# huzaifakhan04/truely-real-time-ai-generated-video-detection-framework-for-social-platforms

Hardware: AMD Instinct MI355X
Metric: frames/sec (detect+embed+drift) 720p (higher is better)
Workload: dtype f32

## Files before the change

### truely-real-time-ai-generated-video-detection-framework-for-social-platforms_amd/csrc/trl_api.hip

```cpp
#include <stdarg.h>
#include <stdio.h>
#include <string.h>
#include <stdlib.h>

#include "trl_ctx.h"

static thread_local char g_err[512] = "";
int g_trl_no_fnconv = 0;
int g_trl_pnet_gate = 0;

#include <mutex>
namespace {
std::mutex g_gate_mu;
hipEvent_t g_gate_ev[64] = {};
bool g_gate_set[64] = {};
}
int trl_gate_wait(trl_ctx* c, hipStream_t s) {
    const int d = c->cfg.device;
    if (!g_trl_pnet_gate || d < 0 || d >= 64) return TRL_OK;
    std::lock_guard<std::mutex> lk(g_gate_mu);
    if (g_gate_set[d]) TRL_HIP(hipStreamWaitEvent(s, g_gate_ev[d], 0));
    return TRL_OK;
}
int trl_gate_record(trl_ctx* c, hipStream_t s) {
    const int d = c->cfg.device;
    if (!g_trl_pnet_gate || d < 0 || d >= 64) return TRL_OK;
    std::lock_guard<std::mutex> lk(g_gate_mu);
    if (!g_gate_ev[d]) TRL_HIP(hipEventCreateWithFlags(&g_gate_ev[d], hipEventDisableTiming));
    TRL_HIP(hipEventRecord(g_gate_ev[d], s));
    g_gate_set[d] = true;
    return TRL_OK;
}
void trl_set_error(const char* fmt, ...) {
    va_list ap;
    va_start(ap, fmt);
    vsnprintf(g_err, sizeof g_err, fmt, ap);
    va_end(ap);
}

extern "C" {

int trl_abi_version(void) { return TRL_ABI_VERSION; }
const char* trl_last_error(void) { return g_err; }

int trl_default_config(trl_config* cfg) {
    if (!cfg) return TRL_ERR_INVALID;
    cfg->device = 0;
    cfg->min_face_size = 20;
    cfg->thr0 = 0.6f; cfg->thr1 = 0.7f; cfg->thr2 = 0.7f;
    cfg->factor = 0.709;
    cfg->cap_level = 2048;
    cfg->cap_frame = 2048;
    cfg->max_faces = 64;
    cfg->pnet_mode = 0;
    cfg->embed_mode = 0;
    cfg->embed_precision = 0;
    return TRL_OK;
}

int trl_create(const trl_config* cfg, trl_ctx** out) {
    if (!cfg || !out) { trl_set_error("null argument"); return TRL_ERR_INVALID; }
    if (cfg->cap_level < 64 || cfg->cap_level > (1 << 24) || cfg->cap_frame < 64 || cfg->cap_frame > (1 << 24) || (cfg->cap_level & 3) ||
        (cfg->cap_frame & 3) || cfg->min_face_size < 12 || cfg->max_faces < 1 || !(cfg->factor > 0.1 && cfg->factor < 0.99) || cfg->embed_mode < 0 || cfg->embed_mode > 3 ||
        cfg->embed_precision < 0 || cfg->embed_precision > 2) {
        trl_set_error("bad trl_config (list start capacities must be multiples of 4 in [64, 2^24], min_face_size >= 12)");
        return TRL_ERR_INVALID;
    }
    TRL_HIP(hipSetDevice(cfg->device));
    trl_ctx* c = new trl_ctx();
    c->cfg = *cfg;
    c->pnet_prof = trl_tune_set("TRL_PNET_CLOCK");
    if (hipMalloc((void**)&c->pnet_clk, 8 * 41) != hipSuccess || hipMemset(c->pnet_clk, 0, 8 * 41) != hipSuccess || hipMemset(c->pnet_clk, 0xFF, 8) != hipSuccess ||
        hipMalloc((void**)&c->pnet_cursor, 64) != hipSuccess || hipHostMalloc((void**)&c->h_pinned, 1024) != hipSuccess ||
        hipEventCreate(&c->ev_call0) != hipSuccess || hipEventCreate(&c->ev_call1) != hipSuccess) {
        trl_set_error("context allocation failed: %s", hipGetErrorString(hipGetLastError()));
        trl_destroy(c);
        return TRL_ERR_HIP;
    }
    memset(c->h_pinned, 0, 1024);
    *out = c;
    return TRL_OK;
}

int trl_destroy(trl_ctx* c) {
    if (!c) return TRL_OK;
    (void)hipSetDevice(c->cfg.device);
    (void)hipDeviceSynchronize();
    c->pend.active = false;
    for (auto& kv : c->W) if (kv.second.pt) (void)hipFree(kv.second.pt);
    if (c->wdev) (void)hipFree(c->wdev);
    if (c->arena.base) (void)hipFree(c->arena.base);
    if (c->scratch.base) (void)hipFree(c->scratch.base);
    if (c->sims_tmp.base) (void)hipFree(c->sims_tmp.base);
    if (c->pyr_tab) (void)hipFree(c->pyr_tab);
    for (auto& b : c->fn_cap) if (b.p) (void)hipFree(b.p);
    if (c->pnet_clk) {
        unsigned long long t[41];
        if (c->pnet_prof && hipMemcpy(t, c->pnet_clk, sizeof t, hipMemcpyDeviceToHost) == hipSuccess && t[2 + 32] > 0) {
            static const char* nm[8] = {"phase0", "barrier0", "phase1", "barrier1", "phase2", "barrier2", "phase3", "barrier3"};
            const double tiles = (double)t[2 + 32];
            fprintf(stderr, "[TRL_PNET_CLOCK] shader clocks per tile (wave 0..3), %.0f workgroup-tiles\n", tiles);
            for (int k = 0; k < 8; k++)
                fprintf(stderr, "[TRL_PNET_CLOCK] %-9s %8.0f %8.0f %8.0f %8.0f\n", nm[k], t[2 + k] / tiles, t[2 + 8 + k] / tiles, t[2 + 16 + k] / tiles, t[2 + 24 + k] / tiles);
            fprintf(stderr, "[TRL_PNET_CLOCK] fp16 screen: %llu M-tiles screened, %llu confirmed (%.2f %%)\n", t[39], t[40],
                    t[39] ? 100.0 * (double)t[40] / (double)t[39] : 0.0);
        }
        (void)hipFree(c->pnet_clk);
    }
    if (c->pnet_cursor) (void)hipFree(c->pnet_cursor);
    if (c->h_pinned) (void)hipHostFree(c->h_pinned);
    if (c->ev_call0) (void)hipEventDestroy(c->ev_call0);
    if (c->ev_call1) (void)hipEventDestroy(c->ev_call1);
    for (auto& e : c->pnet_ev) { (void)hipEventDestroy(e.first); (void)hipEventDestroy(e.second); }
    delete c;
    return TRL_OK;
}

}

namespace {
struct Entry {
    char name[56];
    uint32_t ndim;
    uint32_t dims[4];
    uint64_t offset;
    uint64_t nbytes;
};
static_assert(sizeof(Entry) == 96, "TRLW entry layout");
}

const DevW* trl_w(trl_ctx* c, const std::string& name) {
    auto it = c->W.find(name);
    if (it == c->W.end()) { trl_set_error("weight matrix '%s' not loaded", name.c_str()); return nullptr; }
    return &it->second;
}
const DevV* trl_v(trl_ctx* c, const std::string& name) {
    auto it = c->V.find(name);
    if (it == c->V.end()) { trl_set_error("weight vector '%s' not loaded", name.c_str()); return nullptr; }
    return &it->second;
}

int trl_ensure(trl_ctx* c, Arena& a, size_t bytes) {
    if (bytes <= a.cap) return TRL_OK;
    const size_t ncap = bytes + (bytes >> 3) + (32u << 20);
    TRL_HIP(hipDeviceSynchronize());
    if (a.base) { TRL_HIP(hipFree(a.base)); a.base = nullptr; a.cap = 0; }
    TRL_HIP(hipMalloc((void**)&a.base, ncap));
    a.cap = ncap;
    a.off = 0;
    if (c->dbg_poison >= 0) TRL_HIP(hipMemset(a.base, c->dbg_poison, ncap));
    return TRL_OK;
}

extern "C" int trl_load_weights(trl_ctx* c, const void* blob, size_t nbytes) {
    if (!c || !blob) { trl_set_error("null argument"); return TRL_ERR_INVALID; }
    const uint8_t* b = (const uint8_t*)blob;
    if (nbytes < 16 || memcmp(b, "TRLW0001", 8) != 0) { trl_set_error("bad weights blob magic"); return TRL_ERR_WEIGHTS; }
    uint32_t nt;
    memcpy(&nt, b + 8, 4);
    if (16 + (size_t)nt * sizeof(Entry) > nbytes) { trl_set_error("truncated weights blob"); return TRL_ERR_WEIGHTS; }
    const Entry* ent = (const Entry*)(b + 16);
    TRL_HIP(hipSetDevice(c->cfg.device));

    struct Pending { std::string name; bool mat; int K, Cout, Kpad, ld, n; size_t off; const float* src; };
    std::vector<Pending> items;
    size_t total = 0;
    auto add_mat = [&](const std::string& name, int K, int Cout, const float* src) {
        Pending p; p.name = name; p.mat = true; p.K = K; p.Cout = Cout; p.Kpad = (K + 15) / 16 * 16; p.ld = (Cout + 31) / 32 * 32;
        p.n = 0; p.src = src; p.off = total;
        total += ((size_t)p.Kpad * p.ld * 4 + 255) & ~(size_t)255;
        items.push_back(p);
    };
    auto add_vec = [&](const std::string& name, int n, const float* src) {
        Pending p; p.name = name; p.mat = false; p.K = p.Cout = p.Kpad = p.ld = 0; p.n = n; p.src = src; p.off = total;
        total += ((size_t)((n + 127) / 128 * 128) * 4 + 255) & ~(size_t)255;
        items.push_back(p);
    };
    std::unordered_map<std::string, const Entry*> idx;
    for (uint32_t i = 0; i < nt; i++) {
        const Entry& e = ent[i];
        if (e.offset > nbytes || e.nbytes > nbytes - e.offset || (e.offset & 3)) { trl_set_error("tensor out of blob bounds"); return TRL_ERR_WEIGHTS; }
        std::string name(e.name, strnlen(e.name, 56));
        const uint64_t elems = e.ndim == 2 ? (uint64_t)e.dims[0] * e.dims[1] : (e.ndim == 1 ? (uint64_t)e.dims[0] : 0);
        if ((e.ndim == 1 || e.ndim == 2) && (elems == 0 || elems > (1ull << 31) || elems * 4 != e.nbytes)) {
            trl_set_error("tensor '%s': shape and byte count disagree", name.c_str());
            return TRL_ERR_WEIGHTS;
        }
        idx[name] = &e;
        const float* src = (const float*)(b + e.offset);
        if (e.ndim == 2) add_mat(name, (int)e.dims[0], (int)e.dims[1], src);
        else if (e.ndim == 1) add_vec(name, (int)e.dims[0], src);
    }
    std::vector<std::vector<float>> keep_alive;
    auto merge_heads = [&](const std::string& net, const std::vector<std::string>& parts) -> int {
        int K = -1, tot = 0;
        for (auto& p : parts) {
            auto it = idx.find(net + "." + p + ".w");
            auto ib = idx.find(net + "." + p + ".b");
            if (it == idx.end() || ib == idx.end()) { trl_set_error("missing head %s.%s", net.c_str(), p.c_str()); return TRL_ERR_WEIGHTS; }
            if (K < 0) K = (int)it->second->dims[0];
            if (K != (int)it->second->dims[0] || ib->second->dims[0] != it->second->dims[1]) {
                trl_set_error("head %s.%s has an unexpected shape", net.c_str(), p.c_str());
                return TRL_ERR_WEIGHTS;
            }
            tot += (int)it->second->dims[1];
        }
        keep_alive.emplace_back((size_t)K * tot);
        keep_alive.emplace_back((size_t)tot);
        std::vector<float>& bias = keep_alive[keep_alive.size() - 1];
        std::vector<float>& wm = keep_alive[keep_alive.size() - 2];
        int col = 0;
        for (auto& p : parts) {
            const Entry* e = idx[net + "." + p + ".w"];
            const Entry* eb = idx[net + "." + p + ".b"];
            const float* src = (const float*)(b + e->offset);
            const float* sb = (const float*)(b + eb->offset);
            const int co = (int)e->dims[1];
            for (int k = 0; k < K; k++) for (int j = 0; j < co; j++) wm[(size_t)k * tot + col + j] = src[(size_t)k * co + j];
            for (int j = 0; j < co; j++) bias[col + j] = sb[j];
            col += co;
        }
        add_mat(net + ".heads.w", K, tot, wm.data());
        add_vec(net + ".heads.b", tot, bias.data());
        return TRL_OK;
    };
    keep_alive.reserve(512);
    auto fuse_bconv = [&](const std::string& out, const std::vector<std::string>& parts) -> int {
        int K = -1, tot = 0;
        for (auto& p : parts) {
            auto it = idx.find(p + ".w");
            if (it == idx.end() || idx.find(p + ".scale") == idx.end() || idx.find(p + ".shift") == idx.end()) {
                trl_set_error("missing tensors of %s", p.c_str());
                return TRL_ERR_WEIGHTS;
            }
            if (K < 0) K = (int)it->second->dims[0];
            if (K != (int)it->second->dims[0]) { trl_set_error("fused convs disagree on K (%s)", p.c_str()); return TRL_ERR_WEIGHTS; }
            tot += (int)it->second->dims[1];
        }
        keep_alive.emplace_back((size_t)K * tot); const size_t iw = keep_alive.size() - 1;
        keep_alive.emplace_back((size_t)tot);      const size_t isc = keep_alive.size() - 1;
        keep_alive.emplace_back((size_t)tot);      const size_t ish = keep_alive.size() - 1;
        int col = 0;
        for (auto& p : parts) {
            const Entry* e = idx[p + ".w"];
            const float* src = (const float*)(b + e->offset);
            const float* ssc = (const float*)(b + idx[p + ".scale"]->offset);
            const float* ssh = (const float*)(b + idx[p + ".shift"]->offset);
            const int co = (int)e->dims[1];
            for (int k = 0; k < K; k++) for (int j = 0; j < co; j++) keep_alive[iw][(size_t)k * tot + col + j] = src[(size_t)k * co + j];
            for (int j = 0; j < co; j++) { keep_alive[isc][col + j] = ssc[j]; keep_alive[ish][col + j] = ssh[j]; }
            col += co;
        }
        add_mat(out + ".w", K, tot, keep_alive[iw].data());
        add_vec(out + ".scale", tot, keep_alive[isc].data());
        add_vec(out + ".shift", tot, keep_alive[ish].data());
        return TRL_OK;
// ... 689 lines not shown
```

### truely-real-time-ai-generated-video-detection-framework-for-social-platforms_amd/csrc/trl_pnet.hip

```cpp
#include "trl_ctx.h"
#include <stdlib.h>
#include <type_traits>

typedef float f32x4 __attribute__((ext_vector_type(4)));
typedef float f32x16 __attribute__((ext_vector_type(16)));
typedef _Float16 f16x8 __attribute__((ext_vector_type(8)));
typedef unsigned u32x4_a4 __attribute__((ext_vector_type(4), aligned(4)));
struct __attribute__((packed, aligned(4))) u32x3_a4 { unsigned x, y, z; };

namespace {

constexpr int TS = 16;
constexpr int IN_T = 2 * TS + 10;
constexpr int P1_T = TS + 4;
constexpr int C2_T = TS + 2;
constexpr int C2_LD = 17;
constexpr int REGION_A = C2_T * C2_T * C2_LD;
constexpr int REGION_B = P1_T * P1_T * 10 + 224;
static_assert(3 * 7 * 256 <= REGION_A, "input tile (+ the 28 overhang pixels of the 7x256 copy) fits region A");
static_assert(P1_T * P1_T * 10 <= REGION_B, "pooled tile fits region B");
constexpr int CARRY_P = P1_T * 4 * 10;
constexpr int CARRY_C = C2_T * 2 * C2_LD;
constexpr int BAND = 3;
constexpr int VCARRY_P = 4 * P1_T * 10;
// ... 491 lines not shown
#pragma unroll
    for (int r = 0; r < 4; r++) WH[r] = a.wh[(((lane >> 2) & 7) + 8 * r) * 32 + 4 * (lane >> 5) + (lane & 3)];
    const float bias2 = a.b2[l15], slope2 = a.s2[l15];
    if (tid < 32) { T3all[tid] = a.b3[tid]; T3all[32 + tid] = a.s3[tid]; if (tid < 8) T3all[64 + tid] = a.bh[tid]; }
    if (tid < 32) { T3all[72 + tid] = a.wh[tid * 32 + 1] - a.wh[tid * 32]; if (tid == 0) T3all[104] = a.bh[1] - a.bh[0]; }
    const float sel2 = trl_prelu_sel(slope2);
    const f32x4 bias2v = {bias2, bias2, bias2, bias2};

    for (int i = tid; i < REGION_A; i += 256) RA[i] = 0.f;
    for (int i = tid; i < REGION_B; i += 256) RB[i] = 0.f;
    __syncthreads();

    const int e2_2 = kq >= 2 ? 170 : 0;
    const int xb = lane >> 2, xj = lane & 3, xdy = xj >> 1, xdx = xj & 1;
    float WC[3][2];
#pragma unroll
    for (int cg = 0; cg < 3; cg++)
#pragma unroll
        for (int h = 0; h < 2; h++) {
            const int k = xb + 16 * h;
            WC[cg][h] = k < 27 ? a.w1[k * 32 + 4 * cg + xj] : (k == 27 ? a.b1[4 * cg + xj] : 0.f);
        }
    float xone = 1.0f;
    asm volatile("" : "+v"(xone));
    const int xcg = xj < 3 ? xj : 2;
    const float sl4[4] = {a.s1[4 * xcg], a.s1[4 * xcg + 1], a.s1[4 * xcg + 2], a.s1[4 * xcg + 3]};
    const int c1x_w = ((2 * wave + xdy) * IN_T + 8 + 2 * xb + xdx) * 3;
    const int c1x_sw = (wave * P1_T + 4 + xb) * 10 + 4 * xj;
    const int c1s_l = ((2 * wave + 8 * xj) * IN_T + 8 + 2 * xb) * 3;
    const int c1s_s = ((wave + 4 * xj) * P1_T + 4 + xb) * 10;

    const int total_tiles = a.tiles_per_frame * a.n_frames;
    const int xcd = blockIdx.x & 7;
    const int chunk = (total_tiles + 7) / 8;
    const int t_begin = xcd * chunk, t_end = (t_begin + chunk < total_tiles) ? t_begin + chunk : total_tiles;

    const int lvl_t0v = lane < a.L ? a.lv[lane < 16 ? lane : 15].tile0 : 0x7fffffff;
    auto sdiv = [](int n, unsigned magic, int d) {
        int q = (int)__umulhi((unsigned)n, magic);
        if (q * d > n) q--;
        if (n - q * d >= d) q++;
        return q;
    };
    struct TileId { int f, l, ty, tx, h, w, oh, ow, tiles_x, pix0, rib, rows; float scale; };
    auto decode = [&](int tile) {
        TileId t;
        const int tpf = __builtin_amdgcn_readfirstlane(a.tiles_per_frame);
        t.f = __builtin_amdgcn_readfirstlane(sdiv(tile, __builtin_amdgcn_readfirstlane(a.tpf_magic), tpf));
        const int tt = tile - t.f * tpf;
        t.l = __popcll(__ballot(tt >= lvl_t0v)) - 1;
        const PLevel& g = a.lv[t.l];
        t.h = g.h; t.w = g.w; t.oh = g.oh; t.ow = g.ow; t.tiles_x = g.tiles_x; t.pix0 = g.pix0; t.scale = g.scale;
        const int tq = tt - g.tile0;
        const int band = sdiv(tq, g.bmagic, BAND * t.tiles_x);
        const int rb = tq - band * (BAND * t.tiles_x);
        t.rows = g.tiles_y - BAND * band < BAND ? g.tiles_y - BAND * band : BAND;
        static_assert(BAND == 2 || BAND == 3, "column of a band position: rb / rows for rows in 1..3");
        t.tx = __builtin_amdgcn_readfirstlane(t.rows == 3 ? (rb * 43691) >> 17 : (t.rows == 2 ? rb >> 1 : rb));
        t.rib = rb - t.tx * t.rows;
        t.ty = BAND * band + t.rib;
        return t;
    };
    const int pin_iy0 = tid / IN_T, pin_ix0 = tid - pin_iy0 * IN_T;
    float4 pre[7];
    auto issue_input = [&](const TileId& t) {
        const TileId& g = t;
        const int gy0 = t.ty * 2 * TS, gx0 = t.tx * 2 * TS;
        const char* srcb = reinterpret_cast<const char*>(a.pyr + (long long)t.f * a.pyr_stride + g.pix0 + (long long)gy0 * g.w + gx0);
        const int w16 = g.w * 12;
        const int hrem = g.h - gy0, wrem = g.w - gx0;
        if (hrem >= IN_T && wrem >= IN_T) {
            const unsigned v0 = (unsigned)(pin_iy0 * w16 + pin_ix0 * 12);
#pragma unroll
            for (int i = 0; i < 7; i++) {
                unsigned vo = v0 + (unsigned)(i * (6 * w16 + 48)) + ((pin_ix0 >= IN_T - 4 * i) ? (unsigned)(w16 - IN_T * 12) : 0u);
                if (i == 6) vo = (tid < IN_T * IN_T - 6 * 256) ? vo : 0u;
                { const f32x3_nt v3 = *reinterpret_cast<const f32x3_nt*>(srcb + vo); pre[i] = make_float4(v3[0], v3[1], v3[2], 0.f); }
            }
        } else {
#pragma unroll
            for (int i = 0; i < 7; i++) {
                const bool wrap = pin_ix0 >= IN_T - 4 * i;
                const int iy = pin_iy0 + 6 * i + (wrap ? 1 : 0), ix = pin_ix0 + 4 * i - (wrap ? IN_T : 0);
                const bool ok = iy < hrem && ix < wrem && (i < 6 || tid < IN_T * IN_T - 6 * 256);
                pre[i] = make_float4(0.f, 0.f, 0.f, 0.f);
                if (ok) { const f32x3_nt v3 = *reinterpret_cast<const f32x3_nt*>(srcb + (unsigned)(iy * w16 + ix * 12)); pre[i] = make_float4(v3[0], v3[1], v3[2], 0.f); }
            }
        }
    };
    typedef float f32x2c __attribute__((ext_vector_type(2)));
    int ctid = tid;
    auto copy_pooled = [&](auto SAVE_T, float* CP) {
        constexpr bool SAVE = decltype(SAVE_T)::value;
        const int q = ctid & 15;
#pragma unroll
        for (int pass = 0; pass < 2; pass++) {
            const int r = (ctid >> 4) + 16 * pass;
            if (q < 10 && (pass == 0 || ctid < 64)) {
                f32x4* t = reinterpret_cast<f32x4*>(RB + r * (P1_T * 10) + (SAVE ? 16 * 10 : 0) + 4 * q);
                f32x4* c = reinterpret_cast<f32x4*>(CP + r * 40 + 4 * q);
                if (SAVE) *c = *t; else *t = *c;
            }
        }
    };
    auto copy_conv2 = [&](auto SAVE_T, float* CC) {
        constexpr bool SAVE = decltype(SAVE_T)::value;
        const int q = ctid & 31;
#pragma unroll
        for (int pass = 0; pass < 3; pass++) {
            const int r = (ctid >> 5) + 8 * pass;
            if (q < 17 && (pass < 2 || ctid < 64)) {
                f32x2c* t = reinterpret_cast<f32x2c*>(RA + r * (C2_T * C2_LD) + (SAVE ? 16 * C2_LD : 0) + 2 * q);
                f32x2c* c = reinterpret_cast<f32x2c*>(CC + r * 34 + 2 * q);
                if (SAVE) *c = *t; else *t = *c;
            }
        }
    };
    auto copy_rows = [&](auto SAVE_T) {
        constexpr bool SAVE = decltype(SAVE_T)::value;
        if (ctid < VCARRY_P / 4) {
            f32x4* t = reinterpret_cast<f32x4*>(RB + (SAVE ? 16 * P1_T * 10 : 0)) + ctid;
            f32x4* c = reinterpret_cast<f32x4*>(VP) + ctid;
            if (SAVE) *c = *t; else *t = *c;
        }
    };
    auto copy_rows2 = [&](auto SAVE_T) {
        constexpr bool SAVE = decltype(SAVE_T)::value;
        static_assert((16 * C2_T * C2_LD) % 4 == 0 && VCARRY_C % 4 == 0, "float4 copies");
        if (ctid < VCARRY_C / 4) {
            f32x4* t = reinterpret_cast<f32x4*>(RA + (SAVE ? 16 * C2_T * C2_LD : 0)) + ctid;
            f32x4* c = reinterpret_cast<f32x4*>(VC) + ctid;
            if (SAVE) *c = *t; else *t = *c;
        }
    };
    __shared__ int next_tile_s;
    int run_len = a.run;
    if (tid == 0) next_tile_s = t_begin + atomicAdd(&a.xcd_next[xcd], run_len);
    __syncthreads();
    int tile = __builtin_amdgcn_readfirstlane(next_tile_s);
    __syncthreads();
    TileId cur = decode(tile < t_end ? tile : 0), nxt = cur;
    if (tile < t_end) issue_input(cur);
    int rot = 0, tile_nxt = tile, run_pos = 0;
    int hs_tile[BAND], vs_tile = -1;
#pragma unroll
    for (int i = 0; i < BAND; i++) hs_tile[i] = -1;
    unsigned long long pt[8] = {0, 0, 0, 0, 0, 0, 0, 0}, pt_last = 0;
    const bool prof = DBG && a.prof != 0;
    auto stamp = [&](int k) {
        if (DBG && prof) { const unsigned long long t = clock64(); pt[k] += t - pt_last; pt_last = t; }
    };
    if (DBG && prof) pt_last = clock64();
    unsigned nscr = 0, ncnf = 0;
    for (; tile < t_end; tile = tile_nxt, cur = nxt, rot++) {
        const int f = cur.f, l = cur.l, ty = cur.ty, tx = cur.tx;
        const TileId& g = cur;
        asm volatile("" : "+v"(ctid));
        const int vrows = (g.oh - ty * TS < TS) ? g.oh - ty * TS : TS;
        const bool carry = tx > 0 && (g.rib == 0 ? hs_tile[0] : (g.rib == 1 ? hs_tile[1] : hs_tile[BAND - 1])) == tile - g.rows;
        const bool vcarry = g.rib > 0 && vs_tile == tile - 1;
        const bool last_of_run = run_pos + 1 >= run_len;
        const bool feeds_next = run_pos + g.rows < run_len && tx + 1 < g.tiles_x;
        const bool feeds_down = !last_of_run && g.rib + 1 < g.rows;
        float* const CP = CP0 + g.rib * (CARRY_P + CARRY_C);
        float* const CC = CP + CARRY_P;
        if (feeds_next) { if (g.rib == 0) hs_tile[0] = tile; else if (g.rib == 1) hs_tile[1] = tile; else hs_tile[BAND - 1] = tile; }
        if (feeds_down) vs_tile = tile;
        int cursor = tile + 1 - t_begin;
        int rem = (t_end - tile - 64 * run_len) >> 7;
        const int next_len = rem < 1 ? 1 : (rem > a.run ? a.run : rem);
        if (tid == 0 && last_of_run) cursor = atomicAdd(&a.xcd_next[xcd], next_len);
        run_pos = last_of_run ? 0 : run_pos + 1;
        run_len = last_of_run ? next_len : run_len;

        stamp(7);
        if (!(dbg_skip & 16)) {
#pragma unroll
        for (int i = 0; i < 7; i++) {
            float* d = RA + 3 * tid + 768 * i;
            d[0] = pre[i].x; d[1] = pre[i].y; d[2] = pre[i].z;
        }
        }
        stamp(0);
        __syncthreads();
        stamp(1);

        if (!(dbg_skip & 2)) {
            const int vy = g.h - 2 - ty * 2 * TS, vx = g.w - 2 - tx * 2 * TS;
            const bool fast = vy >= 2 * P1_T && vx >= 2 * P1_T;
            if (carry) copy_pooled(std::false_type{}, CP);
            if (vcarry) copy_rows(std::false_type{});
            struct XU { int lb, sb, row, col; };
            auto wide_u = [&](int i) { XU u; u.lb = c1x_w + i * (8 * IN_T * 3); u.sb = c1x_sw + i * (4 * P1_T * 10); u.row = wave + 4 * i; u.col = 4 + xb; return u; };
            auto narrow_u = [&](int n) {
                XU u; u.row = 4 * n + (xb >> 2); u.col = xb & 3;
                u.lb = ((2 * u.row + xdy) * IN_T + 2 * u.col + xdx) * 3; u.sb = (u.row * P1_T + u.col) * 10 + 4 * xj;
                return u;
            };
            auto x_epi = [&](auto EDGE_T, const XU& u, const f32x4 (&acc)[3]) {
                constexpr bool EDGE = decltype(EDGE_T)::value;
                const float ninf = -__builtin_inff();
                const bool pv = !EDGE || ((2 * u.row + xdy < vy) && (2 * u.col + xdx < vx));
                float m[3][4], n[3][4];
#pragma unroll
                for (int cg = 0; cg < 3; cg++) {
                    f32x4 v = acc[cg];
                    if (EDGE) { v[0] = pv ? v[0] : ninf; v[1] = pv ? v[1] : ninf; v[2] = pv ? v[2] : ninf; v[3] = pv ? v[3] : ninf; }
                    quad_max4(v, m[cg]);
                    if (NEG1) {
                        f32x4 w = acc[cg];
                        if (EDGE) { w[0] = pv ? w[0] : -ninf; w[1] = pv ? w[1] : -ninf; w[2] = pv ? w[2] : -ninf; w[3] = pv ? w[3] : -ninf; }
                        quad_min4(w, n[cg]);
                    }
                }
                const bool cv = !EDGE || ((2 * u.row < vy) && (2 * u.col < vx));
                float o[4];
#pragma unroll
                for (int r = 0; r < 4; r++) {
                    const float pm = lane_sel(lane_sel(m[2][r], m[1][r], 0x2222222222222222ull), m[0][r], 0x1111111111111111ull);
                    const float sel = UNIT ? 0.f : trl_prelu_sel(sl4[r]);
                    if (NEG1) {
                        const float pn = lane_sel(lane_sel(n[2][r], n[1][r], 0x2222222222222222ull), n[0][r], 0x1111111111111111ull);
                        o[r] = prelu_pooled_t<UNIT>(pm, pn, sl4[r], sel);
                    } else {
                        o[r] = prelu_t<UNIT>(pm, sl4[r], sel);
                    }
                    if (EDGE) o[r] = cv ? o[r] : 0.f;
                }
                if (xj < 3) {
                    *reinterpret_cast<f32x2c*>(RB + u.sb) = f32x2c{o[0], o[1]};
                    if (xj < 2) *reinterpret_cast<f32x2c*>(RB + u.sb + 2) = f32x2c{o[2], o[3]};
                }
            };
            auto x_units = [&](auto EDGE_T, auto HASB_T, const XU& A, const XU& B) {
                constexpr bool HASB = decltype(HASB_T)::value;
                f32x4 accA[3], accB[3];
                float xa[2][9], xc[2][9];
                auto rd = [&](int t, float* xo, int lb) {
#pragma unroll
                    for (int u = 0; u < 9; u++) xo[u] = RA[lb + 126 * t + u];
                };
                rd(0, xa[0], A.lb);
                if (HASB) rd(0, xc[0], B.lb);
                const f32x4 z = {0.f, 0.f, 0.f, 0.f};
#pragma unroll
                for (int cg = 0; cg < 3; cg++) {
                    accA[cg] = mfma4<4, 11>(WC[cg][1], xone, z);
                    if (HASB) accB[cg] = mfma4<4, 11>(WC[cg][1], xone, z);
                }
                pn_static_for(std::make_integer_sequence<int, 3>{}, [&](auto T) __attribute__((always_inline)) {
                    constexpr int t = decltype(T)::value;
                    if (t < 2) { rd(t + 1, xa[(t + 1) & 1], A.lb); if (HASB) rd(t + 1, xc[(t + 1) & 1], B.lb); }
                    __builtin_amdgcn_sched_barrier(0);
                    pn_static_for(std::make_integer_sequence<int, 9>{}, [&](auto UU) __attribute__((always_inline)) {
                        constexpr int u = decltype(UU)::value, k = 9 * t + u;
#pragma unroll
                        for (int cg = 0; cg < 3; cg++) {
                            accA[cg] = mfma4<4, (k & 15)>(WC[cg][k >> 4], xa[t & 1][u], accA[cg]);
                            if (HASB) accB[cg] = mfma4<4, (k & 15)>(WC[cg][k >> 4], xc[t & 1][u], accB[cg]);
                        }
                    });
                    __builtin_amdgcn_sched_barrier(0);
                });
                x_epi(EDGE_T, A, accA);
                if (HASB) x_epi(EDGE_T, B, accB);
            };
            auto x_super = [&](auto EDGE_T) {
                constexpr bool EDGE = decltype(EDGE_T)::value;
                const float ninf = -__builtin_inff();
                const int srow = wave + 4 * xj + (vcarry ? 4 : 0), scol = 4 + xb;
                const int sv_l = vcarry ? 8 * IN_T * 3 : 0, sv_s = vcarry ? 4 * P1_T * 10 : 0;
                f32x4 mx[3], mn[3];
                pn_static_for(std::make_integer_sequence<int, 2>{}, [&](auto PP) __attribute__((always_inline)) {
                    constexpr int pp = decltype(PP)::value;
                    const int lbA = c1s_l + sv_l + pp * (IN_T * 3), lbB = lbA + 3;
                    f32x4 accA[3], accB[3];
                    float xa[2][9], xc[2][9];
                    auto rd = [&](int t, float* xo, int lb) {
#pragma unroll
                        for (int u = 0; u < 9; u++) xo[u] = RA[lb + 126 * t + u];
                    };
                    rd(0, xa[0], lbA); rd(0, xc[0], lbB);
                    const f32x4 z = {0.f, 0.f, 0.f, 0.f};
#pragma unroll
                    for (int cg = 0; cg < 3; cg++) { accA[cg] = mfma4<4, 11>(WC[cg][1], xone, z); accB[cg] = mfma4<4, 11>(WC[cg][1], xone, z); }
                    pn_static_for(std::make_integer_sequence<int, 3>{}, [&](auto T) __attribute__((always_inline)) {
                        constexpr int t = decltype(T)::value;
                        if (t < 2) { rd(t + 1, xa[(t + 1) & 1], lbA); rd(t + 1, xc[(t + 1) & 1], lbB); }
                        __builtin_amdgcn_sched_barrier(0);
                        pn_static_for(std::make_integer_sequence<int, 9>{}, [&](auto UU) __attribute__((always_inline)) {
                            constexpr int u = decltype(UU)::value, k = 9 * t + u;
#pragma unroll
                            for (int cg = 0; cg < 3; cg++) {
                                accA[cg] = mfma4<4, (k & 15)>(WC[cg][k >> 4], xa[t & 1][u], accA[cg]);
                                accB[cg] = mfma4<4, (k & 15)>(WC[cg][k >> 4], xc[t & 1][u], accB[cg]);
                            }
                        });
                        __builtin_amdgcn_sched_barrier(0);
                    });
                    const bool pvA = !EDGE || ((2 * srow + pp < vy) && (2 * scol < vx)), pvB = !EDGE || ((2 * srow + pp < vy) && (2 * scol + 1 < vx));
#pragma unroll
                    for (int cg = 0; cg < 3; cg++)
#pragma unroll
                        for (int r = 0; r < 4; r++) {
                            const float va = EDGE ? (pvA ? accA[cg][r] : ninf) : accA[cg][r], vb = EDGE ? (pvB ? accB[cg][r] : ninf) : accB[cg][r];
                            mx[cg][r] = pp == 0 ? vmax_nc(va, vb) : vmax3_nc(mx[cg][r], va, vb);
// ... 85 lines not shown
                        if (hasB) RA[(yB * C2_T + 2 + kq * 4 + q) * C2_LD + l15] = prelu_t<UNIT>(accB[q], slope2, sel2);
                    }
                }
            } else {
            const int c0 = r0 * C2_T, nmt2 = vcarry ? 18 : 21;
            auto read_pair2 = [&](int j) {
                const int mtA = w2 + 8 * j, mtB = (mtA + 4 < 21) ? mtA + 4 : mtA;
                int mA = c0 + mtA * 16 + l15; mA = mA < 324 ? mA : 323;
                int mB = c0 + mtB * 16 + l15; mB = mB < 324 ? mB : 323;
                const int yA = mA / C2_T, xA = mA - yA * C2_T, yB = mB / C2_T, xB = mB - yB * C2_T;
                const int baseA = (yA * P1_T + xA) * 10, baseB = (yB * P1_T + xB) * 10;
#pragma unroll
                for (int s = 0; s < 23; s++) xa[s] = RB[baseA + koff<30, 170>(s, kq, 0, e2_2, 0)];
                if (j < 2 || w2 == 0) {
#pragma unroll
                    for (int s = 0; s < 23; s++) xb[s] = RB[baseB + koff<30, 170>(s, kq, 0, e2_2, 0)];
                }
            };
            read_pair2(0);
#pragma unroll
            for (int j = 0; j < 3; j++) {
                const int mtA = w2 + 8 * j, mtB = mtA + 4;
                const bool hasB = mtB < nmt2 && c0 + 16 * mtB < lim2;
                const bool hasA = mtA < nmt2 && c0 + 16 * mtA < lim2;
                f32x4 accA = bias2v, accB = bias2v;
                __builtin_amdgcn_sched_barrier(0);
                if (!hasA) {
                } else if (hasB) {
                    accA = __builtin_amdgcn_mfma_f32_16x16x4f32(xa[0], B2[0], bias2v, 0, 0, 0);
                    accB = __builtin_amdgcn_mfma_f32_16x16x4f32(xb[0], B2[0], bias2v, 0, 0, 0);
#pragma unroll
                    for (int s = 1; s < 23; s++) {
                        accA = __builtin_amdgcn_mfma_f32_16x16x4f32(xa[s], B2[s], accA, 0, 0, 0);
                        accB = __builtin_amdgcn_mfma_f32_16x16x4f32(xb[s], B2[s], accB, 0, 0, 0);
                    }
                } else {
                    accA = __builtin_amdgcn_mfma_f32_16x16x4f32(xa[0], B2[0], bias2v, 0, 0, 0);
#pragma unroll
                    for (int s = 1; s < 23; s++) accA = __builtin_amdgcn_mfma_f32_16x16x4f32(xa[s], B2[s], accA, 0, 0, 0);
                }
                __builtin_amdgcn_sched_barrier(0);
                if (j < 2) read_pair2(j + 1);
                __builtin_amdgcn_sched_barrier(0);
#pragma unroll
                for (int q = 0; q < 4; q++) {
                    const int ra = c0 + mtA * 16 + kq * 4 + q;
                    if (hasA && ra < 324) RA[ra * C2_LD + l15] = prelu_t<UNIT>(accA[q], slope2, sel2);
                    const int rb = c0 + mtB * 16 + kq * 4 + q;
                    if (hasB && rb < 324) RA[rb * C2_LD + l15] = prelu_t<UNIT>(accB[q], slope2, sel2);
                }
            }
            }
        }
        if (tid == 0) next_tile_s = t_begin + cursor;
        stamp(4);
        __syncthreads();
        stamp(5);

        tile_nxt = __builtin_amdgcn_readfirstlane(next_tile_s);
        if (tile_nxt < t_end) { nxt = decode(tile_nxt); if (!(dbg_skip & 1)) issue_input(nxt); }
        auto strips_get = [&]() __attribute__((always_inline)) {
            if (feeds_next) copy_conv2(std::true_type{}, CC);
            if (feeds_down) copy_rows2(std::true_type{});
        };

        if (!(dbg_skip & 8)) {
            const float fscale = g.scale;
            const f32x4* T3 = reinterpret_cast<const f32x4*>(T3all);
            auto conv3 = [&](int mt, f32x16& P, auto&& between) __attribute__((always_inline)) {
                const int y = mt * 2 + (l31 >> 4), x = l31 & 15;
                const int base = (y * C2_T + x) * C2_LD + hh;
                f32x16 acc;
#pragma unroll
                for (int qa = 0; qa < 4; qa++) {
                    const f32x4 b4 = T3[2 * qa + hh];
                    acc[4 * qa] = b4[0]; acc[4 * qa + 1] = b4[1]; acc[4 * qa + 2] = b4[2]; acc[4 * qa + 3] = b4[3];
                }
                float xa[2][12], wb[2][12];
                auto read_sixth = [&](int sx, float* xo, float* wo) {
#pragma unroll
                    for (int u = 0; u < 12; u++) {
                        const int s = sx * 12 + u, tap = s >> 3, ky = tap / 3, kx = tap - ky * 3;
                        xo[u] = RA[base + (ky * C2_T + kx) * C2_LD + 2 * (s & 7)];
                        wo[u] = B3S[(2 * s + hh) * 32 + l31];
                    }
                };
                read_sixth(0, xa[0], wb[0]);
                pn_static_for(std::make_integer_sequence<int, 6>{}, [&](auto SX) __attribute__((always_inline)) {
                    constexpr int sx = decltype(SX)::value;
                    if (sx < 5) read_sixth(sx + 1, xa[(sx + 1) & 1], wb[(sx + 1) & 1]);
                    __builtin_amdgcn_sched_barrier(0);
                    pn_static_for(std::make_integer_sequence<int, 12>{}, [&](auto UU) __attribute__((always_inline)) {
                        constexpr int u = decltype(UU)::value;
                        acc = __builtin_amdgcn_mfma_f32_32x32x2f32(wb[sx & 1][u], xa[sx & 1][u], acc, 0, 0, 0);
                        between(SX, UU);
                    });
                    __builtin_amdgcn_sched_barrier(0);
                });
#pragma unroll
                for (int qa = 0; qa < 4; qa++) {
                    const f32x4 s4 = T3[8 + 2 * qa + hh];
#pragma unroll
                    for (int qb = 0; qb < 4; qb++) P[4 * qa + qb] = prelu_t<UNIT>(acc[4 * qa + qb], s4[qb], UNIT ? 0.f : trl_prelu_sel(s4[qb]));
                }
            };
            unsigned hlo[4], hhi[4];
            auto head_step = [&](auto H_T, const f32x16& P, f32x4& hq) __attribute__((always_inline)) {
                constexpr int k = decltype(H_T)::value, ga = k >> 3, gb = k & 7;
                if constexpr (gb == 0) {
#pragma unroll
                    for (int qb = 0; qb < 4; qb++) {
                        const unsigned v = __float_as_uint(P[4 * ga + qb]);
                        const auto r = __builtin_amdgcn_permlane32_swap(v, v, false, false);
                        hlo[qb] = r[0]; hhi[qb] = r[1];
                    }
                }
                const float bk = __uint_as_float(gb < 4 ? hlo[gb & 3] : hhi[gb & 3]);
                hq = __builtin_amdgcn_mfma_f32_4x4x1f32(WH[ga], bk, hq, 3, gb, 0);
            };
            auto heads_all = [&](const f32x16& P, f32x4& hq) __attribute__((always_inline)) {
                pn_static_for(std::make_integer_sequence<int, 32>{}, [&](auto H_T) __attribute__((always_inline)) { head_step(H_T, P, hq); });
            };
            auto emit = [&](int mt, const f32x4& hq) __attribute__((always_inline)) {
                if (__builtin_amdgcn_ballot_w64(lane < 32 && hq[1] - hq[0] >= a.dthr) == 0) return;
                const float p = trl_softmax2_p1(hq[0], hq[1]);
                const auto u2 = __builtin_amdgcn_permlane32_swap(__float_as_uint(hq[0]), __float_as_uint(hq[0]), false, false);
                const auto u3 = __builtin_amdgcn_permlane32_swap(__float_as_uint(hq[1]), __float_as_uint(hq[1]), false, false);
                if (lane < 32) {
                    const int oy = ty * TS + mt * 2 + (lane >> 4), ox = tx * TS + (lane & 15);
                    if (oy < g.oh && ox < g.ow) {
                        if (p >= a.thr && !(dbg_skip & 32)) {
                            const int seg = f * a.L + l;
                            const int sl = atomicAdd(&a.lvl_cnt[seg], 1);
                            if (sl < a.lv[l].cap) {
                                Cand c;
                                c.x1 = floorf((2.f * (float)ox + 1.f) / fscale);
                                c.y1 = floorf((2.f * (float)oy + 1.f) / fscale);
                                c.x2 = floorf((2.f * (float)ox + 12.f) / fscale);
                                c.y2 = floorf((2.f * (float)oy + 12.f) / fscale);
                                c.score = p;
                                c.r0 = hq[2]; c.r1 = hq[3]; c.r2 = __uint_as_float(u2[1]); c.r3 = __uint_as_float(u3[1]);
                                c.cell = oy * g.ow + ox;
                                a.lvl_rec[(size_t)f * a.rec_stride + a.lv[l].rec0 + sl] = c;
                            } else {
                                a.flags[0] = 1;
                            }
                        }
                    }
                }
            };
            const int mt0 = wave, mt1 = wave + 4;
            const bool has0 = 2 * mt0 < vrows, has1 = 2 * mt1 < vrows;
            bool cf0 = has0, cf1 = has1;
            if (has0 && a.screen) {
                const int sb0 = ((mt0 * 2 + (l31 >> 4)) * C2_T + (l31 & 15)) * C2_LD + 8 * hh;
                auto screen = [&](int mt, int sb) __attribute__((always_inline)) {
                    f32x16 S;
#pragma unroll
                    for (int qa = 0; qa < 4; qa++) {
                        const f32x4 b4 = T3[2 * qa + hh];
#pragma unroll
                        for (int qb = 0; qb < 4; qb++) S[4 * qa + qb] = b4[qb];
                    }
                    float xm = 0.f;
#pragma unroll
                    for (int tap = 0; tap < 9; tap++) {
                        const int to = ((tap / 3) * C2_T + tap % 3) * C2_LD;
                        f16x8 wv, xv;
#pragma unroll
                        for (int j = 0; j < 8; j++) {
                            wv[j] = (_Float16)B3S[(tap * 16 + 8 * hh + j) * 32 + l31];
                            const float v = RA[sb + to + j];
                            xm = fmaxf(xm, fabsf(v));
                            xv[j] = (_Float16)v;
                        }
                        S = __builtin_amdgcn_mfma_f32_32x32x16_f16(wv, xv, S, 0, 0, 0);
                    }
                    float part = 0.f;
#pragma unroll
                    for (int qa = 0; qa < 4; qa++) {
                        const f32x4 s4 = T3[8 + 2 * qa + hh], w4 = T3[18 + 2 * qa + hh];
#pragma unroll
                        for (int qb = 0; qb < 4; qb++)
                            part = __builtin_fmaf(w4[qb], prelu_t<UNIT>(S[4 * qa + qb], s4[qb], UNIT ? 0.f : trl_prelu_sel(s4[qb])), part);
                    }
                    const auto pp = __builtin_amdgcn_permlane32_swap(__float_as_uint(part), __float_as_uint(part), false, false);
                    const auto px = __builtin_amdgcn_permlane32_swap(__float_as_uint(xm), __float_as_uint(xm), false, false);
                    const float d = (part + __uint_as_float(pp[1])) + T3all[104];
                    const float X = fmaxf(xm, __uint_as_float(px[1]));
                    const float E = __builtin_fmaf(a.scrA, X, a.scrB);
                    const int oy = ty * TS + mt * 2 + (lane >> 4), ox = tx * TS + (lane & 15);
                    const bool hit = !(d + E < a.dthr) || !(fabsf(d) <= 3.402823466e38f) || X > 65504.f;
                    return __builtin_amdgcn_ballot_w64(lane < 32 && oy < g.oh && ox < g.ow && hit) != 0;
                };
                cf0 = screen(mt0, sb0);
                if (has1) cf1 = screen(mt1, sb0 + 8 * C2_T * C2_LD);
                if (DBG) { nscr += has1 ? 2 : 1; ncnf += (cf0 ? 1 : 0) + (cf1 ? 1 : 0); }
            }
            if (cf0 && cf1) {
                f32x16 P0;
                f32x4 hq0 = T3[16 + hh];
                conv3(mt0, P0, [](auto, auto) {});
                {
                    f32x16 P1;
                    f32x4 hq1 = T3[16 + hh];
                    conv3(mt1, P1, [&](auto SX, auto UU) __attribute__((always_inline)) {
                        constexpr int sx = decltype(SX)::value, u = decltype(UU)::value, h = sx * 6 + (u >> 1);
                        if constexpr ((u & 1) == 1 && h < 32) {
                            __builtin_amdgcn_sched_barrier(0);
                            head_step(std::integral_constant<int, h>{}, P0, hq0);
                            __builtin_amdgcn_sched_barrier(0);
                        }
                    });
                    strips_get();
                    heads_all(P1, hq1);
                    emit(mt0, hq0);
                    emit(mt1, hq1);
                }
            } else if (cf0 || cf1) {
                const int mt = cf0 ? mt0 : mt1;
                f32x16 P0;
                f32x4 hq0 = T3[16 + hh];
                conv3(mt, P0, [](auto, auto) {});
                strips_get();
                heads_all(P0, hq0);
                emit(mt, hq0);
            } else {
                strips_get();
            }
        } else {
            strips_get();
        }
        stamp(6);
        __syncthreads();
        stamp(7);
    }
    if (DBG && prof && lane == 0) {
#pragma unroll
        for (int k = 0; k < 8; k++) atomicAdd(&a.clk[2 + 8 * wave + k], pt[k]);
        if (wave == 0) atomicAdd(&a.clk[2 + 32], (unsigned long long)rot);
    }
    if (DBG && lane == 0 && nscr) { atomicAdd(&a.clk[39], (unsigned long long)nscr); atomicAdd(&a.clk[40], (unsigned long long)ncnf); }
    if (DBG && tid == 0) atomicMax(&a.clk[1], (unsigned long long)wall_clock64());
}

}

__global__ void k_pnet_span(unsigned long long* clk) {
    const unsigned long long t0 = clk[0], t1 = clk[1];
    const unsigned long long d = t1 > t0 ? t1 - t0 : 0ull;
    clk[36] += d; clk[37] += 1ull; clk[38] = d;
    clk[0] = ~0ull; clk[1] = 0ull;
}

static int pnet_screen_bound(trl_ctx* c, const DevW* w3, const DevW* wh) {
    std::vector<float> W(144 * 32), H(32 * 32), b3(32), s3(32), bh(8);
    TRL_HIP(hipMemcpy(W.data(), w3->p, W.size() * sizeof(float), hipMemcpyDeviceToHost));
    TRL_HIP(hipMemcpy(H.data(), wh->p, H.size() * sizeof(float), hipMemcpyDeviceToHost));
    TRL_HIP(hipMemcpy(b3.data(), trl_v(c, "pnet.conv3.b")->p, 32 * sizeof(float), hipMemcpyDeviceToHost));
    TRL_HIP(hipMemcpy(s3.data(), trl_v(c, "pnet.prelu3")->p, 32 * sizeof(float), hipMemcpyDeviceToHost));
    TRL_HIP(hipMemcpy(bh.data(), trl_v(c, "pnet.heads.b")->p, 2 * sizeof(float), hipMemcpyDeviceToHost));
    c->pnet_screen_ok = 0; c->pnet_scrA = c->pnet_scrB = __builtin_inff();
    for (float v : W) if (!(fabsf(v) <= 65504.f)) return TRL_OK;
    const double u = ldexp(1.0, -24), uh = ldexp(1.0, -11), tiny = ldexp(1.0, -14);
    auto gamma = [](int n, double uu) { return n * uu / (1.0 - n * uu); };
    const double ge = gamma(145, u), gs = gamma(145, 2 * u), g35 = gamma(35, u), g36 = gamma(36, u);
    double Sa = 0, Sb = fabs((double)bh[0]) + fabs((double)bh[1]);
    double ad = 0, bd = 0, wdP_a = 0, wdP_b = 0;
    for (int co = 0; co < 32; co++) {
        double W1 = 0, D = 0;
        for (int k = 0; k < 144; k++) {
            const double w = W[k * 32 + co], aw = fabs(w);
            W1 += aw;
            D += aw < tiny ? aw : fabs((double)(float)(_Float16)W[k * 32 + co] - w);
        }
        const double b = fabs((double)b3[co]), L = fmax(1.0, fabs((double)s3[co]));
        const double a3 = D * (1 + uh) + W1 * uh + gs * (W1 + D) * (1 + uh) + ge * W1;
        const double b3e = D * tiny + W1 * tiny + gs * (b + (W1 + D) * tiny) + ge * b;
        const double aM = W1 * (1 + ge), bM = b * (1 + ge);
        const double ap = L * (1 + u) * a3 + 2 * u * L * aM, bp = L * (1 + u) * b3e + 2 * u * L * bM;
        const double aP = L * (1 + u) * aM, bP = L * (1 + u) * bM;
        const double w0 = H[co * 32 + 0], w1 = H[co * 32 + 1], wd = fabs(w1 - w0);
        Sa += (fabs(w0) + fabs(w1)) * aP; Sb += (fabs(w0) + fabs(w1)) * bP;
        ad += wd * ap; bd += wd * bp;
        wdP_a += wd * (aP + ap); wdP_b += wd * (bP + bp);
    }
    ad += g36 * (1 + u) * wdP_a;
    bd += g36 * (1 + u) * (fabs((double)bh[1] - (double)bh[0]) + wdP_b);
    const double A = (g35 * Sa + ad) * (1 + ldexp(1.0, -10)), B = (g35 * Sb + bd) * (1 + ldexp(1.0, -10));
    auto up = [](double v) { float f = (float)v; return (double)f < v ? nextafterf(f, __builtin_inff()) : f; };
    c->pnet_scrA = up(A); c->pnet_scrB = up(B); c->pnet_screen_ok = 1;
    return TRL_OK;
}

int trl_pnet_prepare(trl_ctx* c) {
    for (const char* n : {"pnet.conv1.w", "pnet.conv2.w", "pnet.conv3.w", "pnet.heads.w"}) {
        const DevW* w = trl_w(c, n);
        if (!w || w->ld != 32) { trl_set_error("PNet weight %s missing or wrong shape", n); return TRL_ERR_WEIGHTS; }
    }
    const DevW *w1 = trl_w(c, "pnet.conv1.w"), *w2 = trl_w(c, "pnet.conv2.w"), *w3 = trl_w(c, "pnet.conv3.w"), *wh = trl_w(c, "pnet.heads.w");
    if (w1->K != 27 || w1->Cout != 10 || w2->K != 90 || w2->Cout != 16 || w3->K != 144 || w3->Cout != 32 || wh->K != 32 || wh->Cout != 6) {
        trl_set_error("PNet weights have unexpected shapes");
        return TRL_ERR_WEIGHTS;
    }
    float sl[10];
    TRL_HIP(hipMemcpy(sl, trl_v(c, "pnet.prelu1")->p, sizeof sl, hipMemcpyDeviceToHost));
    c->pnet_mono1 = 1;
    for (float v : sl) if (!(v >= 0.f)) c->pnet_mono1 = 0;
    c->pnet_unit = 1;
    for (const char* n : {"pnet.prelu1", "pnet.prelu2", "pnet.prelu3"}) {
        const DevV* v = trl_v(c, n);
        std::vector<float> h(v->n);
        TRL_HIP(hipMemcpy(h.data(), v->p, h.size() * sizeof(float), hipMemcpyDeviceToHost));
        for (float x : h) if (!(x <= 1.f)) c->pnet_unit = 0;
    }
    return pnet_screen_bound(c, w3, wh);
}

static unsigned sdiv_magic(int d) { return d <= 1 ? 0xFFFFFFFFu : (unsigned)((0x100000000ull + (unsigned)d - 1) / (unsigned)d); }

static int fill_args(trl_ctx* c, int n, int H, int W, PnetArgs& a, std::vector<uint32_t>* tab = nullptr) {
    const int L = trl_compute_levels(c, H, W);
    if (L > 16) { trl_set_error("more than 16 pyramid levels"); return TRL_ERR_INVALID; }
    if (L < 1) { trl_set_error("frame %dx%d has no pyramid level at min_face_size %d", W, H, c->cfg.min_face_size); return TRL_ERR_INVALID; }
    a.n_frames = n; a.L = L; a.H = H; a.W = W;
    int tiles = 0, ntab = 0; long long pix = 0, work = 0;
    for (int l = 0; l < L; l++) {
        const LevelGeom& g = c->lv[l];
        PLevel& p = a.lv[l];
        p.h = g.h; p.w = g.w; p.oh = g.oh; p.ow = g.ow;
        p.tiles_x = (g.ow + TS - 1) / TS;
        p.txmagic = sdiv_magic(p.tiles_x);
        p.tile0 = tiles;
        p.tiles_y = (g.oh + TS - 1) / TS;
        p.bmagic = sdiv_magic(BAND * p.tiles_x);
        tiles += p.tiles_x * ((g.oh + TS - 1) / TS);
        p.pix0 = (int)pix;
        p.pix_pad = (int)(((long long)g.h * g.w + 63) & ~63ll);
        pix += p.pix_pad;
        const int khmax = (H + g.h - 1) / g.h + 1, kwmax = (W + g.w - 1) / g.w + 1;
        p.khA = (H + g.h - 1) / g.h; p.kwA = (W + g.w - 1) / g.w;
        p.khmax = (H % g.h) ? p.khA + 1 : p.khA; p.kwmax = (W % g.w) ? p.kwA + 1 : p.kwA;
        p.rkh[0] = 1.0f / (float)p.khA; p.rkh[1] = 1.0f / (float)(p.khA + 1);
        p.rkw[0] = 1.0f / (float)p.kwA; p.rkw[1] = 1.0f / (float)(p.kwA + 1);
        p.fastdiv = (p.khA + 1 <= 96 && p.kwA + 1 <= 96) ? 1 : 0;
        for (int d = 0; d < 4; d++) {
            auto vb = [](int rel, int nbytes) { int hi = nbytes - rel; hi = hi < 0 ? 0 : (hi > 4 ? 4 : hi); return hi >= 4 ? 0xFFFFFFFFu : ((1u << (8 * hi)) - 1u); };
            p.vmA[d] = vb(4 * d, 3 * p.kwA); p.vmB[d] = vb(4 * d, 3 * (p.kwA + 1));
        }
        p.wmagic = (unsigned)((0x100000000ull + g.w - 1) / g.w);
        p.hmagic = (unsigned)((0x100000000ull + g.h - 1) / g.h);
        p.arith = ((unsigned long long)(H + 1) * g.h * g.h < 0x100000000ull && (unsigned long long)(W + 1) * g.w * g.w < 0x100000000ull &&
                   g.h > 1 && g.w > 1) ? 1 : 0;
        p.nd = 3; p.grshift = 0;
        if (kwmax * 3 <= 15 && khmax <= 5) {
            p.mode = 0; p.gshift = 0; p.nd = kwmax * 3 <= 9 ? 3 : 4;
        } else if ((W * 3) % 4 == 0) {
            p.mode = 1;
            const int ngr = (kwmax * 3 + 3 + 11) / 12;
            while ((1 << p.grshift) < ngr) p.grshift++;
            int rlsh = 0;
            while ((khmax >> rlsh) > 8 && p.grshift + rlsh < 6) rlsh++;
            p.gshift = p.grshift + rlsh;
            if (p.gshift > 6) { p.mode = 2; p.gshift = 6; }
        } else {
            p.mode = 2;
            const int dwords = khmax * ((kwmax * 3 + 6) / 4);
            p.gshift = dwords <= 40 ? 0 : (dwords <= 160 ? 2 : (dwords <= 640 ? 4 : 6));
        }
        p.work0 = (int)work;
        work += (long long)p.pix_pad << p.gshift;
        p.ytab0 = ntab; ntab += g.h;
        p.xtab0 = ntab; ntab += g.w;
        if (tab) {
            for (int i = 0; i < g.h; i++) tab->push_back((uint32_t)(((long long)i * H) / g.h) | ((uint32_t)((((long long)i + 1) * H + g.h - 1) / g.h) << 16));
            for (int i = 0; i < g.w; i++) tab->push_back((uint32_t)(((long long)i * W) / g.w) | ((uint32_t)((((long long)i + 1) * W + g.w - 1) / g.w) << 16));
        }
        p.scale = (float)g.scale;
        p.cap = c->cb.lay.capl[l]; p.rec0 = c->cb.lay.rec0[l];
    }
    a.tiles_per_frame = tiles;
    a.tpf_magic = sdiv_magic(tiles);
    a.pyr_stride = pix;
    a.work_per_frame = work;
    a.w1 = trl_w(c, "pnet.conv1.w")->p; a.w2 = trl_w(c, "pnet.conv2.w")->p; a.w3 = trl_w(c, "pnet.conv3.w")->p; a.wh = trl_w(c, "pnet.heads.w")->p;
    a.b1 = trl_v(c, "pnet.conv1.b")->p; a.b2 = trl_v(c, "pnet.conv2.b")->p; a.b3 = trl_v(c, "pnet.conv3.b")->p; a.bh = trl_v(c, "pnet.heads.b")->p;
    a.s1 = trl_v(c, "pnet.prelu1")->p; a.s2 = trl_v(c, "pnet.prelu2")->p; a.s3 = trl_v(c, "pnet.prelu3")->p;
    a.thr = c->cfg.thr0; a.rec_stride = c->cb.lay.S;
    a.dthr = (a.thr >= 0.01f && a.thr <= 0.99f) ? (float)(log((double)a.thr / (1.0 - (double)a.thr)) - 0.05) : -__builtin_inff();
    a.scrA = c->pnet_scrA; a.scrB = c->pnet_scrB; a.screen = c->pnet_screen && c->pnet_screen_ok;
    a.dbg_skip = trl_tune_int("TRL_PNET_SKIP", 0);
    a.lvl_cnt = c->cb.lvl_cnt; a.lvl_rec = c->cb.lvl_rec; a.flags = c->cb.flags;
    a.clk = c->pnet_clk; a.prof = c->pnet_prof ? 1 : 0;
    a.xcd_next = c->pnet_cursor;
    return TRL_OK;
// ... 591 lines not shown
```

Baseline: 20570.

## Pre-convert screen inputs to fp16 in LDS once and batch both M-tiles per tap

Before the fp16 screen, each wave converts its conv2 output cells once into an fp16 staging area in LDS along with per-cell abs-max values, instead of converting eight floats per tap per screen call. The screen then runs both M-tiles in one loop, sharing the weight vector per tap and issuing two independent MFMAs. This removes the per-lane permlane abs-max reduction and the redundant conversions. It also adds optional clock profiling of the screen section. The cost is extra LDS traffic and a wave barrier, and the staging reuses pooled-tile LDS that phase 1 later overwrites.

```diff
diff --git a/truely-real-time-ai-generated-video-detection-framework-for-social-platforms_amd/csrc/trl_api.hip b/truely-real-time-ai-generated-video-detection-framework-for-social-platforms_amd/csrc/trl_api.hip
--- a/truely-real-time-ai-generated-video-detection-framework-for-social-platforms_amd/csrc/trl_api.hip
+++ b/truely-real-time-ai-generated-video-detection-framework-for-social-platforms_amd/csrc/trl_api.hip
@@ -70,7 +70,7 @@
     trl_ctx* c = new trl_ctx();
     c->cfg = *cfg;
     c->pnet_prof = trl_tune_set("TRL_PNET_CLOCK");
-    if (hipMalloc((void**)&c->pnet_clk, 8 * 41) != hipSuccess || hipMemset(c->pnet_clk, 0, 8 * 41) != hipSuccess || hipMemset(c->pnet_clk, 0xFF, 8) != hipSuccess ||
+    if (hipMalloc((void**)&c->pnet_clk, 8 * 45) != hipSuccess || hipMemset(c->pnet_clk, 0, 8 * 45) != hipSuccess || hipMemset(c->pnet_clk, 0xFF, 8) != hipSuccess ||
         hipMalloc((void**)&c->pnet_cursor, 64) != hipSuccess || hipHostMalloc((void**)&c->h_pinned, 1024) != hipSuccess ||
         hipEventCreate(&c->ev_call0) != hipSuccess || hipEventCreate(&c->ev_call1) != hipSuccess) {
         trl_set_error("context allocation failed: %s", hipGetErrorString(hipGetLastError()));
@@ -95,13 +95,14 @@
     if (c->pyr_tab) (void)hipFree(c->pyr_tab);
     for (auto& b : c->fn_cap) if (b.p) (void)hipFree(b.p);
     if (c->pnet_clk) {
-        unsigned long long t[41];
+        unsigned long long t[45];
         if (c->pnet_prof && hipMemcpy(t, c->pnet_clk, sizeof t, hipMemcpyDeviceToHost) == hipSuccess && t[2 + 32] > 0) {
             static const char* nm[8] = {"phase0", "barrier0", "phase1", "barrier1", "phase2", "barrier2", "phase3", "barrier3"};
             const double tiles = (double)t[2 + 32];
             fprintf(stderr, "[TRL_PNET_CLOCK] shader clocks per tile (wave 0..3), %.0f workgroup-tiles\n", tiles);
             for (int k = 0; k < 8; k++)
                 fprintf(stderr, "[TRL_PNET_CLOCK] %-9s %8.0f %8.0f %8.0f %8.0f\n", nm[k], t[2 + k] / tiles, t[2 + 8 + k] / tiles, t[2 + 16 + k] / tiles, t[2 + 24 + k] / tiles);
+            fprintf(stderr, "[TRL_PNET_CLOCK] %-9s %8.0f %8.0f %8.0f %8.0f   (of phase3: the fp16 screen)\n", "screen", t[41] / tiles, t[42] / tiles, t[43] / tiles, t[44] / tiles);
             fprintf(stderr, "[TRL_PNET_CLOCK] fp16 screen: %llu M-tiles screened, %llu confirmed (%.2f %%)\n", t[39], t[40],
                     t[39] ? 100.0 * (double)t[40] / (double)t[39] : 0.0);
         }
diff --git a/truely-real-time-ai-generated-video-detection-framework-for-social-platforms_amd/csrc/trl_pnet.hip b/truely-real-time-ai-generated-video-detection-framework-for-social-platforms_amd/csrc/trl_pnet.hip
--- a/truely-real-time-ai-generated-video-detection-framework-for-social-platforms_amd/csrc/trl_pnet.hip
+++ b/truely-real-time-ai-generated-video-detection-framework-for-social-platforms_amd/csrc/trl_pnet.hip
@@ -667,6 +667,7 @@
     };
     if (DBG && prof) pt_last = clock64();
     unsigned nscr = 0, ncnf = 0;
+    unsigned long long scr_clk = 0;
     for (; tile < t_end; tile = tile_nxt, cur = nxt, rot++) {
         const int f = cur.f, l = cur.l, ty = cur.ty, tx = cur.tx;
         const TileId& g = cur;
@@ -1058,30 +1059,35 @@
             const int mt0 = wave, mt1 = wave + 4;
             const bool has0 = 2 * mt0 < vrows, has1 = 2 * mt1 < vrows;
             bool cf0 = has0, cf1 = has1;
+            const unsigned long long scr_t0 = DBG && prof ? clock64() : 0ull;
             if (has0 && a.screen) {
-                const int sb0 = ((mt0 * 2 + (l31 >> 4)) * C2_T + (l31 & 15)) * C2_LD + 8 * hh;
-                auto screen = [&](int mt, int sb) __attribute__((always_inline)) {
-                    f32x16 S;
-#pragma unroll
-                    for (int qa = 0; qa < 4; qa++) {
-                        const f32x4 b4 = T3[2 * qa + hh];
-#pragma unroll
-                        for (int qb = 0; qb < 4; qb++) S[4 * qa + qb] = b4[qb];
-                    }
-                    float xm = 0.f;
-#pragma unroll
-                    for (int tap = 0; tap < 9; tap++) {
-                        const int to = ((tap / 3) * C2_T + tap % 3) * C2_LD;
-                        f16x8 wv, xv;
+                f16x8* const XH = reinterpret_cast<f16x8*>(RB);
+                float* const CM = RB + C2_T * C2_T * 8;
+                static_assert(C2_T * C2_T * 9 <= P1_T * P1_T * 10, "XH + CM stay inside the pooled rows phase 1 rewrites");
+                const int ln = ctid & 63, ch = ln >> 5;
+                const int ncell = has1 ? 144 : 72;
+#pragma unroll
+                for (int p = 0; p < 3; p++) {
+                    const int i = ln + 64 * p;
+                    if (i < ncell) {
+                        const int cell = 36 * wave + i + (i >= 72 ? 72 : 0);
+                        const float* src = RA + cell * C2_LD;
+                        float m = 0.f;
+                        f16x8 h0, h1;
 #pragma unroll
                         for (int j = 0; j < 8; j++) {
-                            wv[j] = (_Float16)B3S[(tap * 16 + 8 * hh + j) * 32 + l31];
-                            const float v = RA[sb + to + j];
-                            xm = fmaxf(xm, fabsf(v));
-                            xv[j] = (_Float16)v;
+                            const float v0 = src[j], v1 = src[8 + j];
+                            m = fmaxf(m, fabsf(v0)); m = fmaxf(m, fabsf(v1));
+                            h0[j] = (_Float16)v0; h1[j] = (_Float16)v1;
                         }
-                        S = __builtin_amdgcn_mfma_f32_32x32x16_f16(wv, xv, S, 0, 0, 0);
-                    }
+                        XH[2 * cell] = h0; XH[2 * cell + 1] = h1; CM[cell] = m;
+                    }
+                }
+                __builtin_amdgcn_fence(__ATOMIC_RELEASE, "wavefront");
+                __builtin_amdgcn_wave_barrier();
+                __builtin_amdgcn_fence(__ATOMIC_ACQUIRE, "wavefront");
+                const int cb0 = (mt0 * 2 + ((ln >> 4) & 1)) * C2_T + (ln & 15);
+                auto decide = [&](int mt, const f32x16& S, float xm) __attribute__((always_inline)) {
                     float part = 0.f;
 #pragma unroll
                     for (int qa = 0; qa < 4; qa++) {
@@ -1091,18 +1097,43 @@
                             part = __builtin_fmaf(w4[qb], prelu_t<UNIT>(S[4 * qa + qb], s4[qb], UNIT ? 0.f : trl_prelu_sel(s4[qb])), part);
                     }
                     const auto pp = __builtin_amdgcn_permlane32_swap(__float_as_uint(part), __float_as_uint(part), false, false);
-                    const auto px = __builtin_amdgcn_permlane32_swap(__float_as_uint(xm), __float_as_uint(xm), false, false);
                     const float d = (part + __uint_as_float(pp[1])) + T3all[104];
-                    const float X = fmaxf(xm, __uint_as_float(px[1]));
+                    const float X = xm;
                     const float E = __builtin_fmaf(a.scrA, X, a.scrB);
                     const int oy = ty * TS + mt * 2 + (lane >> 4), ox = tx * TS + (lane & 15);
                     const bool hit = !(d + E < a.dthr) || !(fabsf(d) <= 3.402823466e38f) || X > 65504.f;
                     return __builtin_amdgcn_ballot_w64(lane < 32 && oy < g.oh && ox < g.ow && hit) != 0;
                 };
-                cf0 = screen(mt0, sb0);
-                if (has1) cf1 = screen(mt1, sb0 + 8 * C2_T * C2_LD);
+                auto screen = [&](auto TWO_T, bool& c0, bool& c1) __attribute__((always_inline)) {
+                    constexpr bool TWO = decltype(TWO_T)::value;
+                    f32x16 S[2];
+#pragma unroll
+                    for (int qa = 0; qa < 4; qa++) {
+                        const f32x4 b4 = T3[2 * qa + hh];
+#pragma unroll
+                        for (int qb = 0; qb < 4; qb++) { S[0][4 * qa + qb] = b4[qb]; S[1][4 * qa + qb] = b4[qb]; }
+                    }
+                    float xm[2] = {0.f, 0.f};
+#pragma unroll
+                    for (int tap = 0; tap < 9; tap++) {
+                        const int to = (tap / 3) * C2_T + tap % 3;
+                        f16x8 wv;
+#pragma unroll
+                        for (int j = 0; j < 8; j++) wv[j] = (_Float16)B3S[(tap * 16 + 8 * hh + j) * 32 + l31];
+#pragma unroll
+                        for (int m = 0; m < (TWO ? 2 : 1); m++) {
+                            const int c = cb0 + 8 * C2_T * m + to;
+                            xm[m] = fmaxf(xm[m], CM[c]);
+                            S[m] = __builtin_amdgcn_mfma_f32_32x32x16_f16(wv, XH[2 * c + ch], S[m], 0, 0, 0);
+                        }
+                    }
+                    c0 = decide(mt0, S[0], xm[0]);
+                    if (TWO) c1 = decide(mt1, S[1], xm[1]);
+                };
+                if (has1) screen(std::true_type{}, cf0, cf1); else screen(std::false_type{}, cf0, cf1);
                 if (DBG) { nscr += has1 ? 2 : 1; ncnf += (cf0 ? 1 : 0) + (cf1 ? 1 : 0); }
             }
+            if (DBG && prof) scr_clk += clock64() - scr_t0;
             if (cf0 && cf1) {
                 f32x16 P0;
                 f32x4 hq0 = T3[16 + hh];
@@ -1147,6 +1178,7 @@
         if (wave == 0) atomicAdd(&a.clk[2 + 32], (unsigned long long)rot);
     }
     if (DBG && lane == 0 && nscr) { atomicAdd(&a.clk[39], (unsigned long long)nscr); atomicAdd(&a.clk[40], (unsigned long long)ncnf); }
+    if (DBG && prof && lane == 0) atomicAdd(&a.clk[41 + wave], scr_clk);
     if (DBG && tid == 0) atomicMax(&a.clk[1], (unsigned long long)wall_clock64());
 }
 
```

After: 20630, median of 6. Within noise of the previous version (+0.3%).
